# papaboo/Bifrost3D

Hardware: AMD Instinct MI355X
Metric: Mrays/sec + ms/frame at 1080p/256spp; per-pixel RMSE vs OptiXRenderer (higher is better)
Workload: dtype f32

## Files before the change

### bifrost3d_amd/csrc/wide8_kernels.h

```cpp
#pragma once

#include "kernels.h"

namespace hipr {

struct Wide8Scene {
    const uint4* slots;
    uint32_t slot_count;
    float grid_min[3], grid_cell[3];
    uint32_t cull_backfaces;
};

constexpr int WIDE8_STACK_SHALLOW = 12;
#ifndef HIPR_WIDE8_WAVES
#define HIPR_WIDE8_WAVES 6
#endif
#ifndef HIPR_WIDE8_SIGN_HITS
#define HIPR_WIDE8_SIGN_HITS 1
#endif
#ifndef HIPR_WIDE8_LEAF_VOTE_NUM
#define HIPR_WIDE8_LEAF_VOTE_NUM 1
#define HIPR_WIDE8_LEAF_VOTE_DEN 2
#endif
#ifndef HIPR_WIDE8_WAVES_LOW
#define HIPR_WIDE8_WAVES_LOW 6
#endif
HD constexpr int wide8_waves_per_simd(int stack_entries) { return stack_entries <= 8 ? HIPR_WIDE8_WAVES_LOW : (stack_entries <= 12 ? HIPR_WIDE8_WAVES : (stack_entries <= 16 ? 5 : 4)); }

__device__ __forceinline__ void record_barycentrics(uint32_t flags, int which, float ru, float rv, float& u, float& v) {
    const float rw = 1.0f - ru - rv;
    const uint32_t su = (flags >> (which == 0 ? 8 : 12)) & 3u, sv = (flags >> (which == 0 ? 10 : 14)) & 3u;
    u = su == 0u ? rw : (su == 1u ? ru : rv);
    v = sv == 0u ? rw : (sv == 1u ? ru : rv);
}

template <int STACK, int MODE, bool INSTRUMENT, bool COVERAGE = true, bool SORTED = false, bool COVERAGE_R8 = false>
__global__ __launch_bounds__(TRACE_BLOCK) __attribute__((amdgpu_waves_per_eu(wide8_waves_per_simd(STACK)))) void k_trace_wide8(DeviceScene sc, Wide8Scene tree, PathState in, float4* hits, ShadowQueue q,
        float4* radiance, const uint32_t* closest_count_ptr, const uint32_t* shadow_count_ptr, uint32_t* work_counter, int refill_below, DeviceCounters* counters,
        const uint32_t* sorted = nullptr) {
    __shared__ uint2 s_stack[STACK * TRACE_BLOCK];
    uint2* stack = s_stack + threadIdx.x;
    const uint32_t n_closest = MODE != TRACE_SHADOW ? *closest_count_ptr : 0u;
    const uint32_t n = n_closest + (MODE != TRACE_CLOSEST ? *shadow_count_ptr : 0u);
    const uint32_t lane = threadIdx.x & 63u;
    const unsigned long long lt = (1ull << lane) - 1ull;
    const uint32_t chunk_size = min(TRACE_CHUNK_MAX, max(64u, (n / (gridDim.x * (TRACE_BLOCK / 64u) * 2u)) & ~63u));

    uint32_t chunk_next = 0, chunk_end = 0;
    uint32_t shard = (blockIdx.x & 7u) * (TRACE_SHARDS / 8u) + ((blockIdx.x >> 3) % (TRACE_SHARDS / 8u));
    bool exhausted = false;

    bool active = false, finished = false;
    bool is_shadow = MODE == TRACE_SHADOW;
    uint32_t ray_index = 0;
    f3 o = {0, 0, 0}, d = {0, 0, 1}, inv = {0, 0, 0}, ood = {0, 0, 0};
    float tmin = 0.0f, tmax = 0.0f;
    float pay_x = 0.0f, pay_y = 0.0f, pay_z = __uint_as_float(HIPR_HIT_MISS);
    uint32_t pay_k = HIPR_NO_TRIANGLE;
    uint32_t octant = 0;
    uint32_t gx = 0, gy = 0;
    uint32_t item = 0;
    bool item_is_leaf = false;
    int sp = 0;
    uint32_t nodes = 0, tris = 0, shadow_nodes = 0, shadow_tris = 0;
    uint32_t diag_node_iterations = 0, diag_node_lanes = 0, diag_triangle_iterations = 0, diag_triangle_lanes = 0, diag_busy_lanes = 0, diag_refills = 0;
    uint32_t diag_pushes = 0, diag_pushes_deep = 0;
    uint32_t diag_records_closest = 0, diag_records_shadow = 0, diag_records_mixed = 0;

    for (;;) {
        if (finished) {
            if (is_shadow) {
                if constexpr (MODE != TRACE_CLOSEST) {
                    float4 acc = radiance[pay_k];
                    acc.x += pay_x; acc.y += pay_y; acc.z += pay_z;
                    radiance[pay_k] = acc;
                }
            } else if constexpr (MODE != TRACE_SHADOW) {
                for (uint32_t li = 0; li < sc.light_count; ++li) {
                    const HiprLight l = load_light_uniform(sc.lights, li);
                    const uint32_t type = l.flags & HIPR_LIGHT_TYPE_MASK;
                    float t = -1e30f;
                    if (type == HIPR_LIGHT_SPHERE) { if (!(l.data[6] > 0.0f)) continue; t = ray_sphere(o, d, L3(l, 3), l.data[6]); }
                    else if (type == HIPR_LIGHT_SPOT) { if (!(l.data[6] > 0.0f)) continue; t = ray_disk(o, d, L3(l, 3), L3(l, 7), l.data[6]); }
                    else continue;
                    if (t > tmin && t < tmax) { tmax = t; pay_x = 0; pay_y = 0; pay_z = __uint_as_float(HIPR_HIT_LIGHT | li); }
                }
                hits[ray_index] = make_float4(tmax, pay_x, pay_y, pay_z);
            }
            finished = false;
        }
        const unsigned long long idle = wave_ballot(!active);
        if (INSTRUMENT && lane == 0 && idle && !exhausted) ++diag_refills;
        if (idle && !exhausted) {
            while (chunk_next >= chunk_end && !exhausted) {
                const uint32_t shard_begin = uint32_t((unsigned long long)n * shard / TRACE_SHARDS);
                const uint32_t shard_end = uint32_t((unsigned long long)n * (shard + 1u) / TRACE_SHARDS);
                uint32_t base = 0;
                if (lane == 0) base = atomicAdd(work_counter + shard * TRACE_SHARD_STRIDE, chunk_size);
                base = __shfl(base, 0);
                if (base < shard_end - shard_begin) { chunk_next = shard_begin + base; chunk_end = min(chunk_next + chunk_size, shard_end); }
                else {
                    const uint32_t my_size = uint32_t((unsigned long long)n * (lane + 1u) / TRACE_SHARDS) - uint32_t((unsigned long long)n * lane / TRACE_SHARDS);
                    const uint32_t claimed = __hip_atomic_load(work_counter + lane * TRACE_SHARD_STRIDE, __ATOMIC_RELAXED, __HIP_MEMORY_SCOPE_AGENT);
                    const unsigned long long open = wave_ballot(claimed < my_size);
                    if (!open) exhausted = true;
                    else {
                        const unsigned long long rotated = shard ? ((open >> shard) | (open << (64u - shard))) : open;
                        shard = (shard + uint32_t(__builtin_ctzll(rotated))) % TRACE_SHARDS;
                    }
                }
            }
            if (chunk_next < chunk_end) {
                const uint32_t idx = chunk_next + __popcll(idle & lt);
                if (!active && idx < chunk_end) {
                    bool dead = false;
                    float4 ro, rdv;
                    if (MODE == TRACE_FUSED) is_shadow = idx >= n_closest;
                    const uint32_t entry = SORTED ? sorted[idx] : idx;
                    if (is_shadow) {
                        if constexpr (MODE != TRACE_CLOSEST) {
                            const uint32_t si = entry - n_closest;
                            ray_index = si;
                            ro = q.o_tmax[si]; rdv = q.d_slot[si];
                            const float4 rr = q.radiance[si];
                            pay_x = rr.x; pay_y = rr.y; pay_z = rr.z;
                            pay_k = __float_as_uint(rdv.w);
                            tmin = 0.0f; tmax = ro.w;
                        }
                    } else if constexpr (MODE != TRACE_SHADOW) {
                        ray_index = entry;
                        const uint2 meta = in.meta[entry];
                        dead = meta.x == HIPR_DEAD_SLOT;
                        pay_k = meta.y;
                        ro = in.o_tmin[entry]; rdv = in.d_pdf[entry];
                        tmin = ro.w; tmax = __builtin_inff();
                        pay_x = pay_y = 0.0f; pay_z = __uint_as_float(HIPR_HIT_MISS);
                    }
                    if (dead) hits[entry] = make_float4(0, 0, 0, __uint_as_float(HIPR_HIT_MISS));
                    else {
                        o = mk3(ro.x, ro.y, ro.z); d = mk3(rdv.x, rdv.y, rdv.z);
                        const f3 sd = {fabsf(d.x) > 1e-20f ? d.x : copysignf(1e-20f, d.x), fabsf(d.y) > 1e-20f ? d.y : copysignf(1e-20f, d.y),
                                       fabsf(d.z) > 1e-20f ? d.z : copysignf(1e-20f, d.z)};
                        inv = {1.0f / sd.x, 1.0f / sd.y, 1.0f / sd.z};
                        ood = o * inv;
                        octant = (inv.x < 0.0f ? 1u : 0u) | (inv.y < 0.0f ? 2u : 0u) | (inv.z < 0.0f ? 4u : 0u);
                        sp = 0;
                        gx = 1u << 24; gy = 1u << 8;
                        item = 0u; item_is_leaf = false;
                        if (tree.slot_count == 0) finished = true;
                        else active = true;
                    }
                }
                chunk_next = min(chunk_next + uint32_t(__popcll(idle)), chunk_end);
            }
        }
        unsigned long long busy = wave_ballot(active);
        if (!busy) {
            if (wave_ballot(finished)) continue;
            if (exhausted) break;
            continue;
        }

        do {
            const bool leaf_mode = active & item_is_leaf;
            const bool node_mode = active & !item_is_leaf;
            const unsigned long long lmask = wave_ballot(leaf_mode), nmask = wave_ballot(node_mode);
            bool advance = false;
            const unsigned long long shadows = INSTRUMENT && MODE == TRACE_FUSED ? wave_ballot(leaf_mode && is_shadow) : 0ull;
            if (INSTRUMENT && lane == 0) {
                const bool leaves = __popcll(lmask) * HIPR_WIDE8_LEAF_VOTE_DEN > __popcll(nmask) * HIPR_WIDE8_LEAF_VOTE_NUM;
                diag_triangle_iterations += leaves; diag_triangle_lanes += leaves ? __popcll(lmask) : 0;
                diag_node_iterations += !leaves; diag_node_lanes += leaves ? 0 : __popcll(nmask);
                diag_busy_lanes += __popcll(lmask | nmask);
                if (MODE == TRACE_FUSED && leaves) {
                    diag_records_closest += shadows == 0ull; diag_records_shadow += shadows == lmask; diag_records_mixed += shadows != 0ull && shadows != lmask;
                }
            }
            if (__popcll(lmask) * HIPR_WIDE8_LEAF_VOTE_DEN > __popcll(nmask) * HIPR_WIDE8_LEAF_VOTE_NUM) {
                if (leaf_mode) {
                    const uint4* rp = tree.slots + 4 * size_t(item);
                    const uint4 r0 = rp[0], r1 = rp[1], r2 = rp[2], r3 = rp[3];
                    const f3 a = mk3(__uint_as_float(r0.x), __uint_as_float(r0.y), __uint_as_float(r0.z));
                    const f3 e1 = mk3(__uint_as_float(r0.w), __uint_as_float(r1.x), __uint_as_float(r1.y));
                    const f3 e2 = mk3(__uint_as_float(r1.z), __uint_as_float(r1.w), __uint_as_float(r2.x));
                    const f3 e3 = mk3(__uint_as_float(r2.y), __uint_as_float(r2.z), __uint_as_float(r2.w));
                    const uint32_t flags = r3.z;
#ifndef HIPR_WIDE8_CULL_CODE
#define HIPR_WIDE8_CULL_CODE 1
#endif
                    const uint32_t cull = HIPR_WIDE8_CULL_CODE && tree.cull_backfaces != 0u ? flags : 0u;
                    const float refuse_a_below = (cull & 4u) ? -__uint_as_float(r3.w) : -__builtin_inff();
                    const float refuse_b_below = (cull & 8u) ? -__uint_as_float(r3.w) : -__builtin_inff();
                    bool testing = true;
                    advance = true;
#pragma unroll
                    for (int which = 0; which < 2; ++which) {
                        const uint32_t id = which == 0 ? r3.x : r3.y;
                        testing = testing & (id != HIPR_LEAF8_NONE);
                        if (testing) {
                            if (INSTRUMENT) { tris += is_shadow ? 0u : 1u; shadow_tris += is_shadow ? 1u : 0u; }
                            TriangleTest test;
                            const f3 first = which == 0 ? e1 : e2, second = which == 0 ? e2 : e3;
                            const bool hit = triangle_inside(a, first, second, o, d, test);
                            float t = 0.0f, by_det = 0.0f;
                            if (wave_any(hit)) { by_det = 1.0f / test.det; t = dot_fma(second, test.q) * by_det; }
                            if constexpr (MODE != TRACE_CLOSEST) {
                                if (is_shadow && hit && t > tmin && t < tmax) {
                                    float coverage = 1.0f;
                                    if (COVERAGE && !(flags >> which & 1u)) {
                                        float u, v;
                                        record_barycentrics(flags, which, test.un * by_det, test.vn * by_det, u, v);
                                        const float4* record = sc.shade_triangles + SHADE_TRIANGLE_QUADS * size_t(id);
                                        const float4 r3 = record[3], r6 = record[6], r7 = record[7];
                                        const float w = 1.0f - u - v;
                                        const f2 uv = mk2(r6.z, r6.w) * u + mk2(r7.x, r7.y) * v + mk2(r6.x, r6.y) * w;
                                        coverage = COVERAGE_R8 ? material_coverage_r8(sc, sc.materials[__float_as_uint(r3.w)], uv) : material_coverage(sc, sc.materials[__float_as_uint(r3.w)], uv);
                                    }
                                    pay_x *= 1.0f - coverage; pay_y *= 1.0f - coverage; pay_z *= 1.0f - coverage;
                                    if (pay_x < 0.0000001f && pay_y < 0.0000001f && pay_z < 0.0000001f) {
                                        pay_x = pay_y = pay_z = 0.0f;
                                        testing = false;
                                        gy = 0u; sp = 0;
                                    }
                                }
                            }
                            if constexpr (MODE != TRACE_SHADOW) {
                                if (!is_shadow && hit) {
                                    float u, v;
                                    record_barycentrics(flags, which, test.un * by_det, test.vn * by_det, u, v);
                                    const float facing = which == 0 ? test.det : __uint_as_float(__float_as_uint(test.det) ^ ((flags & 16u) << 27));
                                    const bool refused = facing < (which == 0 ? refuse_a_below : refuse_b_below);
                                    const bool closer = !refused & (id != pay_k) & (t > tmin) & ((t < tmax) | ((t == tmax) & (id < __float_as_uint(pay_z))));
                                    tmax = closer ? t : tmax; pay_x = closer ? u : pay_x; pay_y = closer ? v : pay_y; pay_z = closer ? __uint_as_float(id) : pay_z;
                                }
                            }
                        }
                    }
                }
            } else if (node_mode) {
                const uint4* np = tree.slots + 4 * size_t(item);
                const uint4 w0 = np[0], w1 = np[1], w2 = np[2], w3 = np[3];
                if (INSTRUMENT) { nodes += is_shadow ? 0u : 1u; shadow_nodes += is_shadow ? 1u : 0u; }
                advance = true;
                const uint32_t mx = w0.x & 0x1FFFFFu, my = (w0.x >> 21) | ((w0.y & 0x3FFu) << 11), mz = (w0.y >> 10) & 0x1FFFFFu;
                const float ox = fmaf(float(mx), tree.grid_cell[0], tree.grid_min[0]), oy = fmaf(float(my), tree.grid_cell[1], tree.grid_min[1]),
                            oz = fmaf(float(mz), tree.grid_cell[2], tree.grid_min[2]);
                const float ax = __uint_as_float((w0.z & 0xFFu) << 23) * inv.x, ay = __uint_as_float(((w0.z >> 8) & 0xFFu) << 23) * inv.y,
                            az = __uint_as_float(((w0.z >> 16) & 0xFFu) << 23) * inv.z;
                const float bx = fmaf(ox, inv.x, -ood.x), by = fmaf(oy, inv.y, -ood.y), bz = fmaf(oz, inv.z, -ood.z);
                const bool px = ax >= 0.0f, py = ay >= 0.0f, pz = az >= 0.0f;
                const uint32_t nx[2] = {px ? w1.x : w2.z, px ? w1.y : w2.w}, fx[2] = {px ? w2.z : w1.x, px ? w2.w : w1.y};
                const uint32_t ny[2] = {py ? w1.z : w3.x, py ? w1.w : w3.y}, fy[2] = {py ? w3.x : w1.z, py ? w3.y : w1.w};
                const uint32_t nz[2] = {pz ? w2.x : w3.z, pz ? w2.y : w3.w}, fz[2] = {pz ? w3.z : w2.x, pz ? w3.w : w2.y};
                uint32_t h = 0u;
#if HIPR_WIDE8_SIGN_HITS
#pragma unroll
                for (int k = 7; k >= 0; --k) {
                    const int word = k >> 2, shift = 8 * (k & 3);
                    const float x0 = fmaf(float((nx[word] >> shift) & 0xFFu), ax, bx), x1 = fmaf(float((fx[word] >> shift) & 0xFFu), ax, bx);
                    const float y0 = fmaf(float((ny[word] >> shift) & 0xFFu), ay, by), y1 = fmaf(float((fy[word] >> shift) & 0xFFu), ay, by);
                    const float z0 = fmaf(float((nz[word] >> shift) & 0xFFu), az, bz), z1 = fmaf(float((fz[word] >> shift) & 0xFFu), az, bz);
                    const float tnear = fmaxf(fmaxf(x0, y0), fmaxf(z0, tmin));
                    const float tfar = fminf(fminf(fminf(x1, y1), z1), tmax);
                    h = __builtin_amdgcn_alignbit(h, __float_as_uint(fmaf(tfar, 1.0000004f, -tnear)), 31u);
                }
                h = ~h & (w0.w >> 24);
#else
#pragma unroll
                for (int k = 0; k < 8; ++k) {
                    const int word = k >> 2, shift = 8 * (k & 3);
                    const float x0 = fmaf(float((nx[word] >> shift) & 0xFFu), ax, bx), x1 = fmaf(float((fx[word] >> shift) & 0xFFu), ax, bx);
                    const float y0 = fmaf(float((ny[word] >> shift) & 0xFFu), ay, by), y1 = fmaf(float((fy[word] >> shift) & 0xFFu), ay, by);
                    const float z0 = fmaf(float((nz[word] >> shift) & 0xFFu), az, bz), z1 = fmaf(float((fz[word] >> shift) & 0xFFu), az, bz);
                    const float tnear = fmaxf(fmaxf(x0, y0), fmaxf(z0, tmin));
                    float tfar = fminf(fminf(x1, y1), z1);
                    tfar = fminf(tfar, tmax) * 1.0000004f;
                    h |= tnear <= tfar ? (1u << k) : 0u;
                }
                h &= w0.w >> 24;
#endif
                h = (octant & 1u) ? (((h & 0x55u) << 1) | ((h >> 1) & 0x55u)) : h;
                h = (octant & 2u) ? (((h & 0x33u) << 2) | ((h >> 2) & 0x33u)) : h;
                h = (octant & 4u) ? (((h & 0x0Fu) << 4) | (h >> 4)) : h;
                if (h) {
                    if (gy & 0xFFu) {
                        stack[sp * TRACE_BLOCK] = make_uint2(gx, gy);
                        if (INSTRUMENT) { ++diag_pushes; diag_pushes_deep += sp >= 8; }
                        ++sp;
                    }
                    gx = w0.w;
                    gy = h | (w0.z >> 24) << 8;
                }
            }
            if (advance) {
                if ((gy & 0xFFu) == 0u && sp > 0) {
                    --sp;
                    const uint2 popped = stack[sp * TRACE_BLOCK];
                    gx = popped.x; gy = popped.y;
                }
                const bool done = (gy & 0xFFu) == 0u;
                const uint32_t p = uint32_t(__builtin_ctz(gy | 0x100u));
                gy = done ? gy : (gy & (gy - 1u));
                const uint32_t position = (p ^ octant) & 7u;
                item_is_leaf = !((gy >> (8u + position)) & 1u);
                item = (gx & 0xFFFFFFu) + uint32_t(__popc((gx >> 24) & ((1u << position) - 1u)));
                active = !done;
                finished = done;
            }
            busy = wave_ballot(active);
        } while (busy && (exhausted || __popcll(busy) >= refill_below));
    }

    if (INSTRUMENT) {
        wave_add(&counters->node_iterations, diag_node_iterations); wave_add(&counters->node_lanes, diag_node_lanes);
        wave_add(&counters->triangle_iterations, diag_triangle_iterations); wave_add(&counters->triangle_lanes, diag_triangle_lanes);
        wave_add(&counters->busy_lanes, diag_busy_lanes); wave_add(&counters->refills, diag_refills);
        wave_add(&counters->pushes, diag_pushes); wave_add(&counters->pushes_past_16, diag_pushes_deep);
        if (MODE == TRACE_FUSED) {
            wave_add(&counters->record_iterations_closest, diag_records_closest); wave_add(&counters->record_iterations_shadow, diag_records_shadow);
            wave_add(&counters->record_iterations_mixed, diag_records_mixed);
        }
        if (MODE != TRACE_SHADOW) { wave_add(&counters->closest_nodes, nodes); wave_add(&counters->closest_triangles, tris); }
        if (MODE != TRACE_CLOSEST) { wave_add(&counters->shadow_nodes, shadow_nodes); wave_add(&counters->shadow_triangles, shadow_tris); }
    }
}

}
```

Measured before the change: 5800.

## Encode traversal state in item word and hoist ray loads before result writeback

Replaces the separate active, finished and leaf booleans with a single packed item word that carries sentinel values and a record bit, which cuts register use and derives the node mask from the busy mask. The refill loads for new rays are issued before the finished-ray writeback so their memory latency can overlap that work. The analytic light test now caches the light count and, when only one analytic light exists, loads it once per wave instead of looping over every light. The slot address math moves to 24-bit multiplies, which caps slot indices, and asm volatile barriers plus canonicalize calls are added to steer the compiler.

```diff
diff --git a/bifrost3d_amd/csrc/wide8_kernels.h b/bifrost3d_amd/csrc/wide8_kernels.h
--- a/bifrost3d_amd/csrc/wide8_kernels.h
+++ b/bifrost3d_amd/csrc/wide8_kernels.h
@@ -33,6 +33,20 @@
     u = su == 0u ? rw : (su == 1u ? ru : rv);
     v = sv == 0u ? rw : (sv == 1u ? ru : rv);
 }
+
+HD bool is_analytic_light(uint32_t flags, float radius) {
+    const uint32_t type = flags & HIPR_LIGHT_TYPE_MASK;
+    return (type == HIPR_LIGHT_SPHERE || type == HIPR_LIGHT_SPOT) && radius > 0.0f;
+}
+HD float analytic_light_distance(const HiprLight& l, f3 o, f3 d) {
+    return (l.flags & HIPR_LIGHT_TYPE_MASK) == HIPR_LIGHT_SPHERE ? ray_sphere(o, d, L3(l, 3), l.data[6]) : ray_disk(o, d, L3(l, 3), L3(l, 7), l.data[6]);
+}
+
+constexpr uint32_t ITEM_RECORD = 0x80000000u, ITEM_FINISHED = 0xFFFFFFFEu, ITEM_IDLE = 0xFFFFFFFFu;
+__device__ __forceinline__ bool item_active(uint32_t item) { return item < ITEM_FINISHED; }
+__device__ __forceinline__ bool item_on_record(uint32_t item) { return int32_t(item) < int32_t(ITEM_FINISHED); }
+__device__ __forceinline__ bool item_on_node(uint32_t item) { return int32_t(item) >= 0; }
+__device__ __forceinline__ const uint4* item_slot(const uint4* slots, uint32_t item) { return (const uint4*)((const char*)slots + __umul24(item, 64u)); }
 
 template <int STACK, int MODE, bool INSTRUMENT, bool COVERAGE = true, bool SORTED = false, bool COVERAGE_R8 = false>
 __global__ __launch_bounds__(TRACE_BLOCK) __attribute__((amdgpu_waves_per_eu(wide8_waves_per_simd(STACK)))) void k_trace_wide8(DeviceScene sc, Wide8Scene tree, PathState in, float4* hits, ShadowQueue q,
@@ -50,7 +64,6 @@
     uint32_t shard = (blockIdx.x & 7u) * (TRACE_SHARDS / 8u) + ((blockIdx.x >> 3) % (TRACE_SHARDS / 8u));
     bool exhausted = false;
 
-    bool active = false, finished = false;
     bool is_shadow = MODE == TRACE_SHADOW;
     uint32_t ray_index = 0;
     f3 o = {0, 0, 0}, d = {0, 0, 1}, inv = {0, 0, 0}, ood = {0, 0, 0};
@@ -59,38 +72,28 @@
     uint32_t pay_k = HIPR_NO_TRIANGLE;
     uint32_t octant = 0;
     uint32_t gx = 0, gy = 0;
-    uint32_t item = 0;
-    bool item_is_leaf = false;
+    uint32_t item = ITEM_IDLE;
     int sp = 0;
     uint32_t nodes = 0, tris = 0, shadow_nodes = 0, shadow_tris = 0;
     uint32_t diag_node_iterations = 0, diag_node_lanes = 0, diag_triangle_iterations = 0, diag_triangle_lanes = 0, diag_busy_lanes = 0, diag_refills = 0;
     uint32_t diag_pushes = 0, diag_pushes_deep = 0;
     uint32_t diag_records_closest = 0, diag_records_shadow = 0, diag_records_mixed = 0;
 
+    uint32_t analytic_lights = 0, held_light_index = 0;
+    if constexpr (MODE != TRACE_SHADOW) {
+        for (uint32_t li = 0; li < sc.light_count; ++li) {
+            const HiprLight l = load_light_uniform(sc.lights, li);
+            if (!is_analytic_light(l.flags, l.data[6])) continue;
+            if (analytic_lights++ == 0) held_light_index = li;
+        }
+    }
+
     for (;;) {
-        if (finished) {
-            if (is_shadow) {
-                if constexpr (MODE != TRACE_CLOSEST) {
-                    float4 acc = radiance[pay_k];
-                    acc.x += pay_x; acc.y += pay_y; acc.z += pay_z;
-                    radiance[pay_k] = acc;
-                }
-            } else if constexpr (MODE != TRACE_SHADOW) {
-                for (uint32_t li = 0; li < sc.light_count; ++li) {
-                    const HiprLight l = load_light_uniform(sc.lights, li);
-                    const uint32_t type = l.flags & HIPR_LIGHT_TYPE_MASK;
-                    float t = -1e30f;
-                    if (type == HIPR_LIGHT_SPHERE) { if (!(l.data[6] > 0.0f)) continue; t = ray_sphere(o, d, L3(l, 3), l.data[6]); }
-                    else if (type == HIPR_LIGHT_SPOT) { if (!(l.data[6] > 0.0f)) continue; t = ray_disk(o, d, L3(l, 3), L3(l, 7), l.data[6]); }
-                    else continue;
-                    if (t > tmin && t < tmax) { tmax = t; pay_x = 0; pay_y = 0; pay_z = __uint_as_float(HIPR_HIT_LIGHT | li); }
-                }
-                hits[ray_index] = make_float4(tmax, pay_x, pay_y, pay_z);
-            }
-            finished = false;
-        }
-        const unsigned long long idle = wave_ballot(!active);
+        const bool finished = item == ITEM_FINISHED;
+        const unsigned long long idle = wave_ballot(!item_active(item));
         if (INSTRUMENT && lane == 0 && idle && !exhausted) ++diag_refills;
+        bool refill = false;
+        uint32_t idx = 0;
         if (idle && !exhausted) {
             while (chunk_next >= chunk_end && !exhausted) {
                 const uint32_t shard_begin = uint32_t((unsigned long long)n * shard / TRACE_SHARDS);
@@ -111,60 +114,95 @@
                 }
             }
             if (chunk_next < chunk_end) {
-                const uint32_t idx = chunk_next + __popcll(idle & lt);
-                if (!active && idx < chunk_end) {
-                    bool dead = false;
-                    float4 ro, rdv;
-                    if (MODE == TRACE_FUSED) is_shadow = idx >= n_closest;
-                    const uint32_t entry = SORTED ? sorted[idx] : idx;
-                    if (is_shadow) {
-                        if constexpr (MODE != TRACE_CLOSEST) {
-                            const uint32_t si = entry - n_closest;
-                            ray_index = si;
-                            ro = q.o_tmax[si]; rdv = q.d_slot[si];
-                            const float4 rr = q.radiance[si];
-                            pay_x = rr.x; pay_y = rr.y; pay_z = rr.z;
-                            pay_k = __float_as_uint(rdv.w);
-                            tmin = 0.0f; tmax = ro.w;
-                        }
-                    } else if constexpr (MODE != TRACE_SHADOW) {
-                        ray_index = entry;
-                        const uint2 meta = in.meta[entry];
-                        dead = meta.x == HIPR_DEAD_SLOT;
-                        pay_k = meta.y;
-                        ro = in.o_tmin[entry]; rdv = in.d_pdf[entry];
-                        tmin = ro.w; tmax = __builtin_inff();
-                        pay_x = pay_y = 0.0f; pay_z = __uint_as_float(HIPR_HIT_MISS);
+                idx = chunk_next + __popcll(idle & lt);
+                refill = !item_active(item) && idx < chunk_end;
+                chunk_next = min(chunk_next + uint32_t(__popcll(idle)), chunk_end);
+            }
+        }
+        float4 acc = make_float4(0, 0, 0, 0);
+        if constexpr (MODE != TRACE_CLOSEST) if (finished && is_shadow) acc = radiance[pay_k];
+        bool new_is_shadow = MODE == TRACE_SHADOW;
+        uint32_t entry = 0;
+        uint2 meta = make_uint2(0u, HIPR_NO_TRIANGLE);
+        float4 ro = make_float4(0, 0, 0, 0), rdv = ro, rr = ro;
+        if (refill) {
+            if (MODE == TRACE_FUSED) new_is_shadow = idx >= n_closest;
+            entry = SORTED ? sorted[idx] : idx;
+            if (new_is_shadow) {
+                if constexpr (MODE != TRACE_CLOSEST) {
+                    const uint32_t si = entry - n_closest;
+                    ro = q.o_tmax[si]; rdv = q.d_slot[si]; rr = q.radiance[si];
+                }
+            } else if constexpr (MODE != TRACE_SHADOW) {
+                meta = in.meta[entry]; ro = in.o_tmin[entry]; rdv = in.d_pdf[entry];
+            }
+        }
+        HiprLight held_light;
+        if constexpr (MODE != TRACE_SHADOW) if (analytic_lights == 1 && wave_any(finished && !is_shadow)) held_light = load_light_uniform(sc.lights, held_light_index);
+        if (finished) {
+            if (is_shadow) {
+                if constexpr (MODE != TRACE_CLOSEST) {
+                    acc.x += pay_x; acc.y += pay_y; acc.z += pay_z;
+                    radiance[pay_k] = acc;
+                }
+            } else if constexpr (MODE != TRACE_SHADOW) {
+                if (analytic_lights == 1) {
+                    const float t = analytic_light_distance(held_light, o, d);
+                    if (t > tmin && t < tmax) { tmax = t; pay_x = 0; pay_y = 0; pay_z = __uint_as_float(HIPR_HIT_LIGHT | held_light_index); }
+                } else if (analytic_lights > 1) {
+                    for (uint32_t li = 0; li < sc.light_count; ++li) {
+                        const HiprLight l = load_light_uniform(sc.lights, li);
+                        if (!is_analytic_light(l.flags, l.data[6])) continue;
+                        const float t = analytic_light_distance(l, o, d);
+                        if (t > tmin && t < tmax) { tmax = t; pay_x = 0; pay_y = 0; pay_z = __uint_as_float(HIPR_HIT_LIGHT | li); }
                     }
-                    if (dead) hits[entry] = make_float4(0, 0, 0, __uint_as_float(HIPR_HIT_MISS));
-                    else {
-                        o = mk3(ro.x, ro.y, ro.z); d = mk3(rdv.x, rdv.y, rdv.z);
-                        const f3 sd = {fabsf(d.x) > 1e-20f ? d.x : copysignf(1e-20f, d.x), fabsf(d.y) > 1e-20f ? d.y : copysignf(1e-20f, d.y),
-                                       fabsf(d.z) > 1e-20f ? d.z : copysignf(1e-20f, d.z)};
-                        inv = {1.0f / sd.x, 1.0f / sd.y, 1.0f / sd.z};
-                        ood = o * inv;
-                        octant = (inv.x < 0.0f ? 1u : 0u) | (inv.y < 0.0f ? 2u : 0u) | (inv.z < 0.0f ? 4u : 0u);
-                        sp = 0;
-                        gx = 1u << 24; gy = 1u << 8;
-                        item = 0u; item_is_leaf = false;
-                        if (tree.slot_count == 0) finished = true;
-                        else active = true;
-                    }
-                }
-                chunk_next = min(chunk_next + uint32_t(__popcll(idle)), chunk_end);
-            }
-        }
-        unsigned long long busy = wave_ballot(active);
+                }
+                hits[ray_index] = make_float4(tmax, pay_x, pay_y, pay_z);
+            }
+            item = ITEM_IDLE;
+        }
+        if (refill) {
+            is_shadow = new_is_shadow;
+            bool dead = false;
+            if (new_is_shadow) {
+                ray_index = entry - n_closest;
+                pay_x = rr.x; pay_y = rr.y; pay_z = rr.z;
+                pay_k = __float_as_uint(rdv.w);
+                tmin = 0.0f; tmax = ro.w;
+            } else {
+                ray_index = entry;
+                uint32_t path_slot = meta.x;
+                asm volatile("" : "+v"(path_slot));
+                dead = path_slot == HIPR_DEAD_SLOT;
+                pay_k = meta.y;
+                tmin = ro.w; tmax = __builtin_inff();
+                pay_x = pay_y = 0.0f; pay_z = __uint_as_float(HIPR_HIT_MISS);
+            }
+            if (dead) hits[entry] = make_float4(0, 0, 0, __uint_as_float(HIPR_HIT_MISS));
+            else {
+                tmin = __builtin_canonicalizef(tmin); tmax = __builtin_canonicalizef(tmax);
+                o = mk3(ro.x, ro.y, ro.z); d = mk3(rdv.x, rdv.y, rdv.z);
+                const f3 sd = {fabsf(d.x) > 1e-20f ? d.x : copysignf(1e-20f, d.x), fabsf(d.y) > 1e-20f ? d.y : copysignf(1e-20f, d.y),
+                               fabsf(d.z) > 1e-20f ? d.z : copysignf(1e-20f, d.z)};
+                inv = {1.0f / sd.x, 1.0f / sd.y, 1.0f / sd.z};
+                ood = o * inv;
+                octant = (inv.x < 0.0f ? 1u : 0u) | (inv.y < 0.0f ? 2u : 0u) | (inv.z < 0.0f ? 4u : 0u);
+                sp = 0;
+                gx = 1u << 24; gy = 1u << 8;
+                item = tree.slot_count == 0 ? ITEM_FINISHED : 0u;
+            }
+        }
+        unsigned long long busy = wave_ballot(item_active(item));
         if (!busy) {
-            if (wave_ballot(finished)) continue;
+            if (wave_ballot(item == ITEM_FINISHED)) continue;
             if (exhausted) break;
             continue;
         }
 
         do {
-            const bool leaf_mode = active & item_is_leaf;
-            const bool node_mode = active & !item_is_leaf;
-            const unsigned long long lmask = wave_ballot(leaf_mode), nmask = wave_ballot(node_mode);
+            const bool leaf_mode = item_on_record(item);
+            const bool node_mode = item_on_node(item);
+            const unsigned long long lmask = wave_ballot(leaf_mode), nmask = busy & ~lmask;
             bool advance = false;
             const unsigned long long shadows = INSTRUMENT && MODE == TRACE_FUSED ? wave_ballot(leaf_mode && is_shadow) : 0ull;
             if (INSTRUMENT && lane == 0) {
@@ -178,7 +216,7 @@
             }
             if (__popcll(lmask) * HIPR_WIDE8_LEAF_VOTE_DEN > __popcll(nmask) * HIPR_WIDE8_LEAF_VOTE_NUM) {
                 if (leaf_mode) {
-                    const uint4* rp = tree.slots + 4 * size_t(item);
+                    const uint4* rp = item_slot(tree.slots, item);
                     const uint4 r0 = rp[0], r1 = rp[1], r2 = rp[2], r3 = rp[3];
                     const f3 a = mk3(__uint_as_float(r0.x), __uint_as_float(r0.y), __uint_as_float(r0.z));
                     const f3 e1 = mk3(__uint_as_float(r0.w), __uint_as_float(r1.x), __uint_as_float(r1.y));
@@ -238,7 +276,7 @@
                     }
                 }
             } else if (node_mode) {
-                const uint4* np = tree.slots + 4 * size_t(item);
+                const uint4* np = item_slot(tree.slots, item);
                 const uint4 w0 = np[0], w1 = np[1], w2 = np[2], w3 = np[3];
                 if (INSTRUMENT) { nodes += is_shadow ? 0u : 1u; shadow_nodes += is_shadow ? 1u : 0u; }
                 advance = true;
@@ -300,14 +338,13 @@
                 }
                 const bool done = (gy & 0xFFu) == 0u;
                 const uint32_t p = uint32_t(__builtin_ctz(gy | 0x100u));
-                gy = done ? gy : (gy & (gy - 1u));
+                gy &= gy - 1u;
                 const uint32_t position = (p ^ octant) & 7u;
-                item_is_leaf = !((gy >> (8u + position)) & 1u);
-                item = (gx & 0xFFFFFFu) + uint32_t(__popc((gx >> 24) & ((1u << position) - 1u)));
-                active = !done;
-                finished = done;
-            }
-            busy = wave_ballot(active);
+                const uint32_t slot = (gx & 0xFFFFFFu) + uint32_t(__popc(__builtin_amdgcn_ubfe(gx, 24u, position)));
+                const uint32_t record = ((gy >> position) & 0x100u) ^ 0x100u;
+                item = done ? ITEM_FINISHED : (slot | record << 23);
+            }
+            busy = wave_ballot(item_active(item));
         } while (busy && (exhausted || __popcll(busy) >= refill_below));
     }
 
```

Result: faster. 6100 (median of 6 runs) (+5.2%).
